# engyasin/EKF-MonoSLAM_for_3D-reconstruction

Hardware: AMD Instinct MI355X
Metric: EKF updates/sec at N features (state dim 14+6N) (higher is better)
Workload: dtype f32 (state, covariance, every accumulation and every other contraction in fp32; the products of the covariance downdate as 3 x bf16 splits of the fp32 operands, six bf16 products per fp32 product: the dropped terms are <= 2^-24 |a||b| in the worst case (2^-28 on average) -- the size of the fp32 prod; 1 GPU; N=1000 inverse-depth features, n=6014, M=N measured per frame, fp32, 1xMI355X (BASELINE configs[2]); features=1000, state_dim=6014, measured_per_frame=1000, camera=conf_kinect.cfg/scale2, frames_per_map=3000, maps=1

## Files before the change

### ekf-monoslam_for_3d-reconstruction_amd/csrc/ekf_capi.hip

```cpp
#include <hip/hip_runtime.h>

#include <algorithm>
#include <array>
#include <climits>
#include <cmath>
#include <cstdint>
#include <cstdio>
#include <cstdlib>
#include <cstring>
#include <map>
#include <mutex>
#include <string>
#include <type_traits>
#include <vector>

#include "../../include/ekf_monoslam.h"
#include "ekf_buffers.hpp"
#include "ekf_feature_table.hpp"
#include "ekf_dense.hpp"
#include "ekf_image.hpp"
#include "ekf_features.hpp"
#include "ekf_syrk6.hpp"
#include "ekf_chain.hpp"
#include "ekf_small.hpp"
// ... 38 lines not shown
  KID_SEED_MASK,
  KID_SEED_RESPONSE,
  KID_SEED_CANDIDATES,
  KID_SEED_SELECT,
  KID_FRAME_UPLOAD,
  KID_FRAME_INGEST,
  KID_FRAME_RECTIFY,
  KID_COUNT
};

static const char* kKernelNames[KID_COUNT] = {
    "predict_camera",  "propagate_strips", "propagate_streaming", "measure",
    "innovation",      "sigma_ht",         "innovation_cov",      "chol_diag",
    "chol_panel",      "chol_trailing",    "state_update",        "downdate_syrk",
    "solve_trmm",      "normalize_quat",  "add_feature",      "compact_transform",   "misc",
    "w_update", "allgather_h", "allgather_s", "allgather_v", "allgather_sigma",
    "seed_mask", "seed_response", "seed_candidates", "seed_select", "frame_upload", "frame_ingest", "frame_rectify"};

static const char* kLaunchNames[EKF_LAUNCH_KINDS] = {
    "downdate_bf16x6", "downdate_f32", "downdate_f32_fused_wu", "downdate_f32_half_tail", "downdate_f32_t64",
    "row_rider", "row_gemv", "row_tile_gemm", "w_update_gemm", "w_recompute",
    "chain_step_launches", "chain_persistent", "solve", "solve_two_groups", "update_oneblock", "update_allinone",
    "chain_trail_diag", "split_image", "state_update_tail", "update_onelaunch", "chain_dist_gather", "chain_step_fused",
    "downdate_mirror_bounds"};

static inline int round_up(int v, int a) { return (v + a - 1) / a * a; }

struct MaskedStreamPool {
  struct Entry { int device, num_cus, reserved; hipStream_t st; };
  std::mutex mu;
  std::vector<Entry> idle;
  bool hooked = false;
  static void at_exit();
  hipStream_t take(int device, int num_cus, int reserved) {
    std::lock_guard<std::mutex> lk(mu);
    for (size_t i = 0; i < idle.size(); ++i)
      if (idle[i].device == device && idle[i].num_cus == num_cus && idle[i].reserved == reserved) {
        hipStream_t st = idle[i].st;
        idle.erase(idle.begin() + i);
        return st;
      }
    return nullptr;
  }
  void give(int device, int num_cus, int reserved, hipStream_t st) {
    std::lock_guard<std::mutex> lk(mu);
    idle.push_back({device, num_cus, reserved, st});
    if (!hooked) { hooked = true; atexit(&MaskedStreamPool::at_exit); }
// ... 169 lines not shown
  bool have_frame = false, have_blur = false;
  DevBuf<unsigned char> d_raw;
  int raw_w = 0, raw_h = 0, raw_c = 0;
  bool have_raw = false;
  RectScratch rect;
  DevBuf<int4> d_ingest_tab;
  int ingest_tab_w = 0, ingest_tab_h = 0;
  DevBuf<unsigned char> d_patch[2], d_mpatch[2];
  int cur_patch = 0;
  DevBuf<T> d_hb, d_zm;
  DevBuf<unsigned char> d_found;
  DevBuf<float> d_score;
  DevBuf<int> d_keep;
  int opt_panel_direct = 1;
  int opt_chain_fused_diag = 1;
  int opt_small_onelaunch = 1;
  int opt_step_fused = 1;
  struct StepPlan { std::vector<int> off, cnt; } sfp;
  WorkList sf_lists{{0}, {}};
  DevBuf<unsigned long long> d_small_stamps;
  unsigned small_gate_total = 0;
  int opt_su_tail = 1;
  int opt_syrk_mirror_skip = 1;
  int opt_fuse_split = 1;
  int opt_chain_defer = 1;
  int td_min_blocks = 24;
  int td_max_blocks = 1 << 30;
  WorkList td_blocks;
  std::vector<int> td_off, td_cnt;
  int opt_syrk_stag_half = 0, opt_syrk_stag_mod4 = 2;
  int opt_solve_s2 = 1;
  bool want_solve_s2(int width, int npad_live) const {
    return kIsF32 && opt_mfma && opt_solve_s2 && (opt_solve_s2 > 1 || (width / 128) * (npad_live / 64) <= 2 * num_cus);
  }
  int opt_fused = 1;
  int opt_solve_one_per_cu = 1;
  int opt_wrecompute = 1;
  int opt_row_gemv = 1;
  int opt_fuse_wu = 1;
  int env_chunks[8] = {}, env_nchunks = 0;
  int opt_pipeline = -1;
  WorkList tilemap{{0, 0}, {}};
  int tri_count = 0, solve_off = 0;
  int w_zeroed_n = -1;
  DevBuf<int> d_counters;
  int num_cus = 256, reserved_cus = 32;
// ... 83 lines not shown
    HIPCHK(d_Hc.reserve(cn * 14));
    HIPCHK(d_Hf.reserve(cn * 12));
    HIPCHK(d_Sd.reserve(cn * 4));
    HIPCHK(d_flags.reserve(cn));
    HIPCHK(d_cflag.reserve(cn));
    HIPCHK(d_trk.reserve(cn));
    HIPCHK(hipMemsetAsync(d_trk, 0, cn, stream));
    HIPCHK(d_Jy.reserve(cn * 18));
    HIPCHK(d_Yxyz.reserve(cn * 3));
    HIPCHK(d_map_src.reserve((size_t)n_pad));
    HIPCHK(d_map_conv.reserve((size_t)n_pad));
    HIPCHK(d_Y.reserve((size_t)2 * ldy * ldy));
    HIPCHK(hipMemsetAsync(d_Y, 0, (size_t)2 * ldy * ldy * sizeof(T), stream));
    HIPCHK(d_W.reserve((size_t)w_rows * ldy));
    HIPCHK(hipMemsetAsync(d_W, 0, (size_t)w_rows * ldy * sizeof(T), stream));
    HIPCHK(d_V.reserve((size_t)w_rows * ldy));
    HIPCHK(hipMemsetAsync(d_V, 0, (size_t)w_rows * ldy * sizeof(T), stream));
    HIPCHK(d_Dinv.reserve((size_t)(ldy / 64) * 128 * 128));
    HIPCHK(d_z.reserve((size_t)ldy));
    HIPCHK(d_midx.reserve(cn));
    HIPCHK(d_status.reserve(16));
    HIPCHK(hipMemsetAsync(d_status, 0, 16 * sizeof(int), stream));
    HIPCHK(d_tmp.reserve(64));
    HIPCHK(d_counters.reserve(kQueueCounters + kMirrorRowsInts));
    HIPCHK(hipMemset(d_counters, 0, (kQueueCounters + kMirrorRowsInts) * sizeof(int)));
    {
      hipDeviceProp_t prop;
      HIPCHK(hipGetDeviceProperties(&prop, device));
      num_cus = prop.multiProcessorCount > 0 ? prop.multiProcessorCount : 256;
    }
    {
      reserved_cus = std::min(32, num_cus / 4);
      if (const char* e = getenv("EKF_RESERVED_CUS")) reserved_cus = std::max(1, std::min(num_cus / 2, atoi(e)));
      std::vector<uint32_t> mask((num_cus + 31) / 32, 0xffffffffu);
      for (int i = 0; i < reserved_cus; ++i) mask[i / 32] &= ~(1u << (i % 32));
      stream_b = g_masked_streams.take(device, num_cus, reserved_cus);
      stream_b_masked = stream_b != nullptr;
      if (!stream_b) {
        if (hipExtStreamCreateWithCUMask(&stream_b, (uint32_t)mask.size(), mask.data()) == hipSuccess) {
          stream_b_masked = true;
        } else {
          (void)hipGetLastError();
          stream_b = nullptr;
          reserved_cus = 0;
          HIPCHK(hipStreamCreateWithFlags(&stream_b, hipStreamNonBlocking));
        }
      }
      stream_b_reserved = reserved_cus;

      if (const char* e = getenv("EKF_FUSE_WU")) opt_fuse_wu = atoi(e);
      if (const char* e = getenv("EKF_ROW_GEMV")) opt_row_gemv = atoi(e) ? 1 : 0;
      if (const char* e = getenv("EKF_SOLVE_ONE_PER_CU")) opt_solve_one_per_cu = atoi(e) ? 1 : 0;
      if (const char* e = getenv("EKF_W_RECOMPUTE")) opt_wrecompute = atoi(e) ? 1 : 0;
      if (const char* e = getenv("EKF_SOLVE_S2")) opt_solve_s2 = atoi(e);
      if (const char* e = getenv("EKF_FUSED_LAUNCHES")) opt_fused = atoi(e) ? 1 : 0;
      if (const char* e = getenv("EKF_PANEL_DIRECT")) opt_panel_direct = atoi(e);
      if (const char* e = getenv("EKF_SYRK_STAGGER")) {
        opt_syrk_stag_half = atoi(e);
        if (const char* c = strchr(e, ',')) opt_syrk_stag_mod4 = atoi(c + 1);
      }
      if (const char* e = getenv("EKF_CHAIN_FUSED_DIAG")) opt_chain_fused_diag = atoi(e) ? 1 : 0;
      if (const char* e = getenv("EKF_FUSE_SPLIT")) opt_fuse_split = atoi(e) ? 1 : 0;
      if (const char* e = getenv("EKF_SU_TAIL")) opt_su_tail = atoi(e) ? 1 : 0;
      if (const char* e = getenv("EKF_SYRK_MIRROR_SKIP")) opt_syrk_mirror_skip = atoi(e) ? 1 : 0;
      if (const char* e = getenv("EKF_SMALL_ONELAUNCH")) opt_small_onelaunch = atoi(e) ? 1 : 0;
      if (const char* e = getenv("EKF_STEP_FUSED")) opt_step_fused = atoi(e) ? 1 : 0;
      if (const char* e = getenv("EKF_SHARD_DIST_CHAIN")) opt_shard_dist_chain = atoi(e) ? 1 : 0;
      if (const char* e = getenv("EKF_SHARD_DIST_MIN_BLOCKS")) shard_dist_min_blocks = std::max(2, atoi(e));
      if (const char* e = getenv("EKF_SMALL_STAMPS")) {
        if (atoi(e)) { HIPCHK(d_small_stamps.reserve(16)); HIPCHK(hipMemset(d_small_stamps, 0, 16 * sizeof(unsigned long long))); }
      }
      if (const char* e = getenv("EKF_CHAIN_DEFER")) opt_chain_defer = atoi(e) ? 1 : 0;
      if (const char* e = getenv("EKF_TD_MIN_BLOCKS")) td_min_blocks = std::max(1, atoi(e));
      if (const char* e = getenv("EKF_TD_MAX_BLOCKS")) td_max_blocks = std::max(1, atoi(e));
      if (const char* e = getenv("EKF_SPLIT_TAIL")) opt_split_tail = atoi(e);
      if (const char* e = getenv("EKF_SPLIT_BF16")) opt_split_bf16 = atoi(e) ? 1 : 0;
      if (const char* e = getenv("EKF_CHUNKS")) {
        for (const char* q = e; *q && env_nchunks < 8;) {
          env_chunks[env_nchunks++] = atoi(q);
          while (*q && *q != ',') ++q;
          if (*q == ',') ++q;
        }
      }
    }
    std::vector<T> mu0(camera_dim, T(0));
    mu0[3] = T(0.0); mu0[4] = T(0.0); mu0[5] = T(-0.707106781); mu0[6] = T(0.707106781);
    if (camera_dim == 14) mu0[13] = T(1);
// ... 788 lines not shown
    if (s2) {
      T* o = static_cast<T*>(s2);
      const T* sd = psd;
      for (int i = 0; i < N; ++i) { o[4 * i] = sd[4 * i]; o[4 * i + 1] = sd[4 * i + 2]; o[4 * i + 2] = sd[4 * i + 1]; o[4 * i + 3] = sd[4 * i + 3]; }
    }
    if (hc) { T* o = static_cast<T*>(hc); for (int i = 0; i < N; ++i) for (int a = 0; a < 2; ++a) for (int c = 0; c < 7; ++c) o[14 * i + c * 2 + a] = vhc[14 * i + a * 7 + c]; }
    if (hf) { T* o = static_cast<T*>(hf); for (int i = 0; i < N; ++i) for (int a = 0; a < 2; ++a) for (int c = 0; c < 6; ++c) o[12 * i + c * 2 + a] = vhf[12 * i + a * 6 + c]; }
    return EKF_OK;
  }

  struct GemmCall {
    const T* A = nullptr; int lda = 0;
    const T* B = nullptr; int ldb = 0;
    T* C = nullptr; int ldc = 0;
    int rows = 0, cols = 0, K = 0;
    T alpha = T(1), beta = T(0);
    int tri = TRI_ALL, row_off = 0, col_off = 0, ktri = KTRI_FULL, ktile_off = 0;
    int zrow = 0, zcol_end = 0;
    const int* tile_list = nullptr; int ntiles = 0;
    int* counter = nullptr;
    void* img = nullptr; int img_nkc = 0, img_c0 = 0;
    bool two_groups = false;
    bool one_per_cu = false;
    hipStream_t st = nullptr;
  };
  struct Rows { int r0, count; };
  struct UpdatePlan {
    int M = 0, plane = 0;
    int nb = 0, tile = 0, m = 0, m_pad = 0, npad_live = 0, nsteps = 0;
    int nchunks = 1, cend[8] = {};
    ChunkTab tab{};
    int strip_rows = 0;
    int ntr = 0, ntc = 0;
    bool oneblock = false, allinone = false, onelaunch = false;
    int small_rc = 0, small_nchunk = 0, small_nt64 = 0;
    bool recompute = false;
    int r0 = 0, r1 = 0, p0 = 0, prows = 0;
    Rows ranges[3] = {};
    bool sym_panel = false, shard_split = false;
    int c0(int g) const { return (g ? cend[g - 1] : 0) * nb; }
    int c1(int g) const { return cend[g] * nb; }
  };
  struct UpdateCtx {
    const T* z;
    const int* midx;
    int* counters;
    int counter_next = 0;
    bool step_fused = false;
    int diag_ahead = -1;
    struct { int step = -1, c0 = 0, c1 = 0; } pending;
    bool row_pending = false;
    bool queue_room(int ints = 8) const { return counter_next + ints <= kQueueCounters; }
    int* take_queue() {
      if (!queue_room()) return nullptr;
      counter_next += 8;
      return counters + counter_next - 8;
    }
  };

  template <int ROLE, bool BT, int TM = 128, int TN = 128>
  void gemm(const GemmCall& c) {
    GemmArgs g{};
    g.A = c.A; g.lda = c.lda; g.B = c.B; g.ldb = c.ldb; g.C = c.C; g.ldc = c.ldc;
    g.K = c.K; g.alpha = double(c.alpha); g.beta = double(c.beta);
    g.tri = c.tri; g.row_off = c.row_off; g.col_off = c.col_off; g.ktri = c.ktri; g.ktile_off = c.ktile_off;
    g.zrow = c.zrow; g.zcol_end = c.zcol_end;
    g.stagger = (ROLE == ROLE_DOWNDATE) ? 1 : 0;
    g.img = c.img; g.img_nkc = c.img_nkc; g.img_c0 = c.img_c0;
    hipStream_t st = c.st ? c.st : stream;
    const bool mf = kIsF32 && opt_mfma;
    dim3 grid(c.cols / (mf ? TN : 64), c.rows / (mf ? TM : 64));
    if (c.tile_list && c.counter) {
      g.tile_map = c.tile_list;
      g.ntiles = c.ntiles;
      g.counter = c.counter;
      const bool side = (st == stream_b);
      int wgs = 2 * (side ? (num_cus - reserved_cus) : num_cus);
      if (ROLE == ROLE_SOLVE && c.one_per_cu) wgs = num_cus;
      grid = dim3(std::min(c.ntiles, wgs), 1);
    }
    if constexpr (kIsF32) {
      if (opt_mfma) {
        if constexpr (ROLE == ROLE_SOLVE) {
          ++launch_cnt[c.two_groups ? EKF_LAUNCH_SOLVE_TWO_GROUPS : EKF_LAUNCH_SOLVE];
          if (c.two_groups) {
            k_gemm_mfma<ROLE, BT, TM, TN, true><<<grid, 512, 0, st>>>(g);
            return;
          }
        }
        k_gemm_mfma<ROLE, BT, TM, TN><<<grid, 256, 0, st>>>(g);
        return;
// ... 133 lines not shown
      *strip_rows = std::max(*strip_rows, (cend[g] - (g ? cend[g - 1] : 0)) * nb);
    }
    return tab;
  }

  int build_innovation(const T* zp, const int* ip, int M, int plane, bool with_nu, int* m_out, int* m_pad_out,
                       const ChunkTab* tab = nullptr, int strip_rows = 0, bool w_only = false) {
    const int nb = NB();
    const int m = 2 * M + (plane ? 3 : 0);
    const int m_pad = round_up(m, nb);
    const int npad_live = round_up(n, nb);
    T* nu_row = d_W + (size_t)ldy * npad_live;
    if (w_zeroed_n != n) {
      HIPCHK(hipMemsetAsync(d_W + (size_t)n * ldy, 0, (size_t)(npad_live - n + nb) * ldy * sizeof(T), stream));
      w_zeroed_n = n;
    }
    const bool small = (size_t)n * m_pad < ((size_t)1 << 22);
    {
      Scope sc(this, KID_SIGMA_HT);
      const int extra = with_nu ? 1 : 0;
      const T* zq = with_nu ? zp : nullptr;
      T* nuq = with_nu ? nu_row : nullptr;
      const ChunkTab st = tab ? *tab : ChunkTab{0, {}};
      int* mrows = (with_nu && tab) ? d_counters + kQueueCounters : nullptr;
      if (small) {
        constexpr int RB = 4;
        dim3 grid((m_pad / 2 + 255) / 256, (n + RB - 1) / RB + extra);
        k_sigma_ht<T, RB><<<grid, 256, 0, stream>>>(S(), ld, n, d_Hc, d_Hf, d_pos, d_coding, ip, M, plane, d_W, ldy,
                                                  m_pad, 0, n, N, zq, d_h, mu(), nuq, d_counters, d_status, d_scr + SCR_QOLD, 0, 0, st, mrows);
      } else if constexpr (kIsF32) {
        constexpr int RB = 8;
        dim3 grid((m_pad / 2 + 127) / 128, (n + RB - 1) / RB + extra);
        k_sigma_ht_fast<RB><<<grid, 256, 0, stream>>>(S(), ld, n, d_Hc, d_Hf, d_pos, d_coding, ip, M, plane, d_W, ldy, m_pad, N,
                                                      0, 0, zq, d_h, mu(), nuq, d_counters, d_status, d_scr + SCR_QOLD, 0, st, mrows);
      } else {
        constexpr int RB = 32;
        dim3 grid((m_pad / 2 + 255) / 256, (n + RB - 1) / RB + extra);
        k_sigma_ht<T, RB><<<grid, 256, 0, stream>>>(S(), ld, n, d_Hc, d_Hf, d_pos, d_coding, ip, M, plane, d_W, ldy,
                                                  m_pad, 0, n, N, zq, d_h, mu(), nuq, d_counters, d_status, d_scr + SCR_QOLD, 0, 0, st, mrows);
      }
    }
    if (!w_only) {
      Scope sc(this, KID_INNOVATION_COV);
      T* zid = tab ? d_Y + (size_t)m_pad * ldy : nullptr;
      const ChunkTab ct = tab ? *tab : ChunkTab{0, {}};
      if (small) {
        constexpr int KB = 1;
// ... 321 lines not shown
        int rc = ensure_step_fused_lists(p.nsteps);
        if (rc) return rc;
        ux.step_fused = true;
      }
    }
    return EKF_OK;
  }

  bool chunk_overlaps(const UpdatePlan& p, int g) const { return stream_b != nullptr && g + 1 < p.nchunks; }
  int chunk_slots(const UpdatePlan& p, int g) const { return 2 * (chunk_overlaps(p, g) ? num_cus - reserved_cus : num_cus); }
  bool chunk_splits(const UpdatePlan& p, const UpdateCtx& ux) const {
    return kIsF32 && opt_split_bf16 && opt_mfma && p.tile == 128 && tri_count >= num_cus && ux.queue_room();
  }
  bool chunk_fuses(const UpdatePlan& p, int g, const UpdateCtx& ux) const {
    return kIsF32 && opt_fuse_wu && (opt_fuse_wu > 1 || p.recompute || g + 2 < p.nchunks) && opt_mfma && chunk_overlaps(p, g) &&
           p.c1(g) < p.m_pad && !opt_split_bf16 && p.tile == 128 && tri_count >= num_cus && ux.queue_room();
  }
  bool chunk_row_rider(const UpdatePlan& p, int g, const UpdateCtx& ux) const {
    return chunk_splits(p, ux) && p.recompute && opt_row_gemv && p.c1(g) < p.m_pad && !chunk_fuses(p, g, ux);
  }
  bool chunk_su_tail(const UpdatePlan& p, int g, const UpdateCtx& ux) const {
    return kIsF32 && opt_su_tail && !chunk_overlaps(p, g) && p.nchunks > 1 && chunk_splits(p, ux);
  }
  enum SolveShape { SOLVE_64X64, SOLVE_128_ONE_PER_CU, SOLVE_64X128, SOLVE_128 };
  SolveShape solve_shape(const UpdatePlan& p, int g) const {
    const bool mf = kIsF32 && opt_mfma;
    const int tiles = (p.c1(g) - p.c0(g)) / p.tile * p.ntr, slots = chunk_slots(p, g);
    if (mf && 4 * tiles < slots) return SOLVE_64X64;
    if (mf && !chunk_overlaps(p, g) && opt_solve_one_per_cu && tiles < slots && tiles > num_cus) return SOLVE_128_ONE_PER_CU;
    if (mf && tiles < slots) return SOLVE_64X128;
    return SOLVE_128;
  }

  int launch_update_small(const UpdatePlan& p, const UpdateCtx& ux) {
    if constexpr (kIsF32) {
      if (w_zeroed_n != n) {
        HIPCHK(hipMemsetAsync(d_W + (size_t)n * ldy, 0, (size_t)(p.npad_live - n + p.nb) * ldy * sizeof(T), stream));
        w_zeroed_n = n;
      }
      SmallUpdateArgs a{};
      a.S = S(); a.ld = ld; a.n = n; a.npad = p.npad_live;
      a.Hc = d_Hc; a.Hf = d_Hf; a.pos = d_pos; a.coding = d_coding; a.midx = ux.midx;
      a.M = p.M; a.plane = p.plane; a.nfeat = N;
      a.z = ux.z; a.h = d_h; a.mu = mu();
      a.r_pix = T(sigma_pixel_2); a.r_plane = T(0.00001);
      a.W = d_W; a.ldw = ldy; a.Y = d_Y; a.ldy = ldy; a.Dinv = d_Dinv; a.V = d_V; a.ldv = ldy;
// ... 11 lines not shown

  int solve_chunk(const UpdatePlan& p, int gi, UpdateCtx& ux, hipStream_t ss, bool* vimg_done) {
    const int c0 = p.c0(gi), width = p.c1(gi) - c0, ntr = p.ntr, ntc = p.ntc;
    T* Zs = d_Y + (size_t)p.m_pad * ldy;
    if (p.oneblock) {
      if constexpr (kIsF32) {
        ++launch_cnt[p.allinone ? EKF_LAUNCH_UPDATE_ALLINONE : EKF_LAUNCH_UPDATE_ONEBLOCK];
        if (p.allinone)
          k_update_oneblock_small<<<p.small_nt64 + 1, 512, 0, ss>>>(d_W, ldy, d_Dinv, d_V, ldy, p.npad_live, mu(), n, d_scr + SCR_QOLD,
                                                                   d_scr + SCR_QN, Zs, ldy, S(), ld, p.small_nt64);
        else
          k_solve_state_oneblock<<<p.npad_live / 64 + 1, 256, 0, ss>>>(d_W, ldy, d_Dinv, d_V, ldy, p.npad_live, mu(), n,
                                                                      d_scr + SCR_QN, Zs, ldy);
      }
      return EKF_OK;
    }
    Scope sc(this, KID_SOLVE, ss);
    const int wt = width / p.tile;
    GemmCall c;
    c.A = d_W + c0; c.lda = ldy; c.B = Zs + c0; c.ldb = ldy; c.C = d_V + c0; c.ldc = ldy;
    c.rows = p.npad_live + p.nb; c.cols = width; c.K = width; c.ktri = KTRI_UPPER;
    c.two_groups = want_solve_s2(width, p.npad_live);
    c.st = ss;
    switch (solve_shape(p, gi)) {
      case SOLVE_64X64:
        c.tile_list = tilemap.d + solve6464_off + 2 * (2 * ntc - 2 * wt) * 2 * ntr; c.ntiles = 2 * wt * 2 * ntr;
        c.counter = ux.take_queue();
        gemm<ROLE_SOLVE, true, 64, 64>(c);
        break;
      case SOLVE_128_ONE_PER_CU:
        c.tile_list = tilemap.d + solve_off + 2 * (ntc - wt) * ntr; c.ntiles = wt * ntr;
        c.counter = ux.take_queue();
        c.one_per_cu = true;
        gemm<ROLE_SOLVE, true>(c);
        break;
      case SOLVE_64X128:
        if (kIsF32 && opt_fuse_split && opt_split_bf16 && p.tile == 128 && tri_count >= num_cus && ux.queue_room(16)) {
          HIPCHK(ensure_vimg());
          c.img = d_Vimg; c.img_nkc = ldy / 16; c.img_c0 = c0;
          *vimg_done = true;
        }
        c.tile_list = tilemap.d + solve64_off + 2 * (ntc - wt) * 2 * ntr; c.ntiles = wt * 2 * ntr;
        c.counter = ux.take_queue();
        gemm<ROLE_SOLVE, true, 64, 128>(c);
        break;
      case SOLVE_128:
// ... 11 lines not shown
    if (p.recompute) {
      launch_row_update(c0, c1, p.m_pad, ss, kIsF32 && opt_row_gemv);
      return;
    }
    Scope sc(this, KID_WUPDATE, ss);
    ++launch_cnt[EKF_LAUNCH_W_UPDATE_GEMM];
    GemmCall c;
    c.A = d_V + c0; c.lda = ldy; c.B = d_Y + (size_t)c1 * ldy + c0; c.ldb = ldy; c.C = d_W + c1; c.ldc = ldy;
    c.rows = p.npad_live + p.nb; c.cols = p.m_pad - c1; c.K = c1 - c0; c.alpha = T(-1); c.beta = T(1);
    c.st = ss;
    if (kIsF32 && opt_mfma && ((p.m_pad - c1) / 128) * p.ntr < chunk_slots(p, gi))
      gemm<ROLE_WUPDATE, false, 64, 128>(c);
    else
      gemm<ROLE_WUPDATE, false>(c);
  }

  int downdate_chunk(const UpdatePlan& p, int gi, UpdateCtx& ux, hipStream_t ss, bool vimg_done) {
    const int c0 = p.c0(gi), c1 = p.c1(gi), width = c1 - c0, m = p.m, m_pad = p.m_pad, npad_live = p.npad_live;
    if (chunk_splits(p, ux)) {
      const bool row_rider = chunk_row_rider(p, gi, ux), su_tail = chunk_su_tail(p, gi, ux);
      if (!vimg_done) ++launch_cnt[EKF_LAUNCH_SPLIT_IMAGE];
      const int* mirror_rows = nullptr;
      if (opt_syrk_mirror_skip && gi + 1 < p.nchunks)
        mirror_rows = d_counters + kQueueCounters + 2 * (p.recompute ? gi + 1 : kMirrorEmpty);
      return launch_downdate_bf16x6(ux, c0, c1, m_pad, ss, !vimg_done, tilemap.d + tri6_off, tri_count, 0, 0, INT_MAX,
                                    double(n) * n * (std::min(c1, m) - std::min(c0, m)), row_rider, su_tail, mirror_rows);
    }
    if (chunk_fuses(p, gi, ux)) {
      if constexpr (kIsF32) {
        Scope sc(this, KID_DOWNDATE, ss);
        const int nr2 = p.recompute ? 1 : (npad_live + p.nb) / 128, n2 = nr2 * ((m_pad - c1) / 128);
        if (sc.on) {
          const double w = std::min(c1, m) - std::min(c0, m);
          prof.work[KID_DOWNDATE] += double(n) * n * w + 2.0 * (p.recompute ? 1 : n + 1) * std::max(0, m - c1) * w;
        }
        GemmArgs g{};
        g.A = d_V + c0; g.lda = ldy; g.B = d_V + c0; g.ldb = ldy; g.C = S(); g.ldc = ld;
        g.K = width; g.alpha = -1.0; g.beta = 1.0; g.tri = TRI_LOWER_MIRROR;
        g.tile_map = tilemap.d; g.ntiles = n2 + tri_count; g.counter = ux.take_queue(); g.stagger = 1;
        g.B2 = d_Y + (size_t)c1 * ldy + c0; g.ldb2 = ldy; g.C2 = d_W + c1; g.ldc2 = ldy;
        g.n2 = n2; g.nr2 = nr2; g.row2 = p.recompute ? npad_live / 128 : 0;
        ++launch_cnt[EKF_LAUNCH_DOWNDATE_F32_FUSED_WU];
        const int wgs = 2 * (num_cus - reserved_cus);
        k_gemm_mfma<ROLE_DOWNDATE, false><<<std::min(g.ntiles, wgs), 256, 0, ss>>>(g);
      }
      return EKF_OK;
    }
// ... 60 lines not shown
    rc = ensure_tilemap(p.npad_live / p.tile, p.ntr, p.ntc);
    if (rc) return rc;
    rc = prepare_chain(p, ux, false);
    if (rc) return rc;
    const int nchunks = p.nchunks, m_pad = p.m_pad;
    bool b_inflight = false;
    for (int gi = 0; gi < (p.onelaunch ? 0 : nchunks); ++gi) {
      const int c0 = p.c0(gi), c1 = p.c1(gi);
      chain_steps(ux, gi ? p.cend[gi - 1] : 0, p.cend[gi], c0, c1, p.m, m_pad, stream, p.oneblock,
                  opt_chain_defer && gi + 1 < nchunks);
      const bool overlap = chunk_overlaps(p, gi);
      hipStream_t ss = overlap ? stream_b : stream;
      if (!overlap && b_inflight) {
        if (p.recompute) {
          HIPCHK(hipEventRecord(ev_b, stream_b));
          HIPCHK(hipStreamWaitEvent(stream, ev_b, 0));
          b_inflight = false;
        } else {
          HIPCHK(hipStreamWaitEvent(stream, ev_wu, 0));
        }
      }
      if (overlap) {
        b_inflight = true;
        HIPCHK(hipEventRecord(ev_chain[gi], stream));
        HIPCHK(hipStreamWaitEvent(stream_b, ev_chain[gi], 0));
      }
      bool vimg_done = false;
      rc = solve_chunk(p, gi, ux, ss, &vimg_done);
      if (rc) return rc;
      const bool fuse = chunk_fuses(p, gi, ux);
      wupdate_chunk(p, gi, ux, ss);
      if (overlap && c1 < m_pad && !fuse && !p.recompute) HIPCHK(hipEventRecord(ev_wu, stream_b));
      if (!overlap && b_inflight) {
        HIPCHK(hipEventRecord(ev_b, stream_b));
        HIPCHK(hipStreamWaitEvent(stream, ev_b, 0));
        b_inflight = false;
      }
      if (!overlap && nchunks > 1 && !chunk_su_tail(p, gi, ux)) {
        HIPCHK(hipEventRecord(ev_chain[gi], stream));
        HIPCHK(hipStreamWaitEvent(stream_b, ev_chain[gi], 0));
        launch_state_update(m_pad, stream_b);
        b_inflight = true;
      }
      rc = downdate_chunk(p, gi, ux, ss, vimg_done);
      if (rc) return rc;
      if (fuse && !p.recompute) HIPCHK(hipEventRecord(ev_wu, stream_b));
      if (p.recompute && gi + 1 < nchunks) {
        launch_w_recompute(c1, p.c1(gi + 1), m_pad, ux.midx, M, plane, ss, n);
// ... 3496 lines not shown
```

### ekf-monoslam_for_3d-reconstruction_amd/csrc/ekf_dense.hpp

```cpp
#pragma once
#include <type_traits>
#include "ekf_math.hpp"

namespace ekf {

typedef float f32x4 __attribute__((ext_vector_type(4)));
constexpr int kQueueCounters = 256;

__device__ __forceinline__ int clamp_feature(int fi, int nfeat) { return min(max(fi, 0), nfeat - 1); }
__device__ __forceinline__ void check_measured_entry(const int* __restrict__ midx, int k, int nfeat,
                                                     int* __restrict__ status) {
  const int fi = midx[k];
  if (status && (fi < 0 || fi >= nfeat || (k > 0 && midx[k - 1] >= fi))) status[1] = 1;
}

struct ChunkTab {
  int n;
  int end[8];
};

constexpr int kMirrorEmpty = 8;
constexpr int kMirrorRowsInts = 2 * (kMirrorEmpty + 1);
__device__ __forceinline__ void mirror_rows_slab(const ChunkTab& tab, const int* __restrict__ midx, int M, int nfeat,
                                                 const int* __restrict__ pos, const int* __restrict__ coding,
                                                 int* __restrict__ mrows) {
  __shared__ int s_lo[8], s_hi[8];
  const int tid = threadIdx.x;
  if (tid < 8) { s_lo[tid] = 0x7fffffff; s_hi[tid] = 0; }
  __syncthreads();
  for (int k = tid; k < M; k += blockDim.x) {
    int g = 0;
#pragma unroll
    for (int u = 0; u < 7; ++u)
      if (u + 1 < tab.n && 2 * k >= tab.end[u]) g = u + 1;
    const int fi = clamp_feature(midx[k], nfeat);
    const int p = pos[fi];
    atomicMin(&s_lo[g], p);
    atomicMax(&s_hi[g], p + (coding[fi] ? 3 : 6));
  }
  __syncthreads();
  if (tid <= kMirrorEmpty) {
    const bool some = tid < 8 && s_hi[tid & 7] > s_lo[tid & 7];
    mrows[2 * tid] = some ? s_lo[tid] : 0;
    mrows[2 * tid + 1] = some ? s_hi[tid] : 0;
  }
}

template <typename T>
__global__ void k_innovation(const T* __restrict__ z, const T* __restrict__ h, const int* __restrict__ midx,
                             int M, int plane, const T* __restrict__ mu, T* __restrict__ nu, int m_pad,
                             int* __restrict__ counters, int nfeat, int* __restrict__ status) {
  const int t = blockIdx.x * blockDim.x + threadIdx.x;
  if (counters)
    for (int c = t; c < kQueueCounters; c += gridDim.x * blockDim.x) counters[c] = 0;
  if (t >= m_pad) return;
  T v = T(0);
  if (t < 2 * M) {
    if ((t & 1) == 0) check_measured_entry(midx, t >> 1, nfeat, status);
    v = z[t] - h[2 * clamp_feature(midx[t >> 1], nfeat) + (t & 1)];
  } else if (plane && t < 2 * M + 3) {
    const int e = t - 2 * M;
    v = -mu[e == 0 ? 1 : (e == 1 ? 4 : 6)];
  }
  nu[t] = v;
}

template <typename T, int RB>
__global__ void k_sigma_ht(const T* __restrict__ S, int ld, int n,
                           const T* __restrict__ Hc, const T* __restrict__ Hf,
                           const int* __restrict__ pos, const int* __restrict__ coding,
                           const int* __restrict__ midx, int M, int plane,
                           T* __restrict__ W, int ldy, int m_pad, int row_begin, int row_end,
                           int nfeat,
                           const T* __restrict__ z = nullptr, const T* __restrict__ h = nullptr,
                           const T* __restrict__ mu = nullptr, T* __restrict__ nu = nullptr,
                           int* __restrict__ counters = nullptr, int* __restrict__ status = nullptr,
                           T* __restrict__ q_old = nullptr, int slot0 = 0, int slot_end = 0,
                           ChunkTab tab = ChunkTab{0, {}}, int* __restrict__ mirror_rows = nullptr) {
  const int k = slot0 + blockIdx.x * blockDim.x + threadIdx.x;
  const int nslots = slot_end > 0 ? slot_end : m_pad / 2;
  if (nu != nullptr && blockIdx.y == gridDim.y - 1) {
    if (q_old && k < 4) q_old[k] = mu[3 + k];
    if (counters)
      for (int c = k; c < kQueueCounters; c += gridDim.x * blockDim.x) counters[c] = 0;
    if (mirror_rows && blockIdx.x == 0) mirror_rows_slab(tab, midx, M, nfeat, pos, coding, mirror_rows);
    if (k >= nslots) return;
    if (k < M) check_measured_entry(midx, k, nfeat, status);
#pragma unroll
    for (int t = 2 * k; t < 2 * k + 2; ++t) {
      T v = T(0);
      if (t < 2 * M) {
        v = z[t] - h[2 * clamp_feature(midx[t >> 1], nfeat) + (t & 1)];
      } else if (plane && t < 2 * M + 3) {
        const int e = t - 2 * M;
        v = -mu[e == 0 ? 1 : (e == 1 ? 4 : 6)];
      }
      nu[t] = v;
    }
    return;
  }
  const int row0 = row_begin + blockIdx.y * RB;
  if (k >= nslots) return;
  const int row1 = min(row0 + RB, min(row_end, n));
  if (k < M) {
    const int fi = clamp_feature(midx[k], nfeat);
    const int p = pos[fi];
    const int fs = coding[fi] ? 3 : 6;
// ... 55 lines not shown

template <int RB>
__global__ void __launch_bounds__(256, RB <= 8 ? 6 : 3)
k_sigma_ht_fast(const float* __restrict__ S, int ld, int n,
                const float* __restrict__ Hc, const float* __restrict__ Hf,
                const int* __restrict__ pos, const int* __restrict__ coding,
                const int* __restrict__ midx, int M, int plane,
                float* __restrict__ W, int ldy, int m_pad, int nfeat, int slot0, int slot_end,
                const float* __restrict__ z, const float* __restrict__ h, const float* __restrict__ mu,
                float* __restrict__ nu, int* __restrict__ counters, int* __restrict__ status, float* __restrict__ q_old,
                int row_lo = 0,
                ChunkTab tab = ChunkTab{0, {}}, int* __restrict__ mirror_rows = nullptr) {
  constexpr int SL = 128, SEG = 6 * SL + 4;
  typedef float f4 __attribute__((ext_vector_type(4)));
  typedef float f2 __attribute__((ext_vector_type(2)));
  __shared__ __attribute__((aligned(16))) float seg[RB * SEG];
  __shared__ __attribute__((aligned(16))) float cam[RB * 8];
  const int tid = threadIdx.x;
  if (nu != nullptr && blockIdx.y == gridDim.y - 1) {
    const int k = blockIdx.x * blockDim.x + tid;
    const int nslots = m_pad / 2;
    if (q_old && k < 4) q_old[k] = mu[3 + k];
    if (counters)
      for (int c = k; c < kQueueCounters; c += gridDim.x * blockDim.x) counters[c] = 0;
    if (mirror_rows && blockIdx.x == 0) mirror_rows_slab(tab, midx, M, nfeat, pos, coding, mirror_rows);
    if (k >= nslots) return;
    if (k < M) check_measured_entry(midx, k, nfeat, status);
#pragma unroll
    for (int t = 2 * k; t < 2 * k + 2; ++t) {
      float v = 0.f;
      if (t < 2 * M) {
        v = z[t] - h[2 * clamp_feature(midx[t >> 1], nfeat) + (t & 1)];
      } else if (plane && t < 2 * M + 3) {
        const int e = t - 2 * M;
        v = -mu[e == 0 ? 1 : (e == 1 ? 4 : 6)];
      }
      nu[t] = v;
    }
    return;
  }
  const int s = tid & (SL - 1), half = tid >> 7;
  const int kbase = slot0 + blockIdx.x * SL;
  const int k = kbase + s;
  const int nslots = slot_end > 0 ? slot_end : m_pad / 2;
  const int row0 = row_lo + blockIdx.y * RB, row1 = min(row0 + RB, n);
  int fi = -1, p = 0, fs = 6;
  if (k < M && k < nslots) {
// ... 173 lines not shown
    }
  }
}

enum : int { ROLE_PANEL = 0, ROLE_TRAILING = 1, ROLE_DOWNDATE = 2, ROLE_SOLVE = 3, ROLE_GAIN = 4, ROLE_WUPDATE = 5 };
enum : int { TRI_ALL = 0, TRI_LOWER = 1, TRI_LOWER_MIRROR = 2, TRI_LISTED = 3 };
enum : int { KTRI_FULL = 0, KTRI_UPPER = 1 };

struct GemmArgs {
  const void* A; int lda;
  const void* B; int ldb;
  void* C; int ldc;
  int K;
  double alpha, beta;
  int tri, row_off, col_off, ktri, ktile_off;
  const int* tile_map; int ntiles; int* counter;
  int zrow, zcol_end;
  int stagger;
  const void* B2; int ldb2;
  void* C2; int ldc2;
  int n2, nr2;
  int row2;
  void* img = nullptr; int img_nkc = 0, img_c0 = 0;
};
constexpr int kSecondProduct = 0x10000;
constexpr int kHalfTile = 0x20000;
constexpr int kMirrorTile = 0x40000;

__device__ __forceinline__ bool gemm_next_tile(const GemmArgs& g, int* s_tile, int& iter, int& bi, int& bj) {
  if (!g.tile_map) {
    if (iter++) return false;
    bi = blockIdx.y;
    bj = blockIdx.x;
    return true;
  }
  __syncthreads();
  if (threadIdx.x == 0) {
    *s_tile = atomicAdd(g.counter, 1);
  }
  __syncthreads();
  const int t = __builtin_amdgcn_readfirstlane(*s_tile);
  if (t >= g.ntiles) return false;
  if (t < g.n2) {
    bi = g.row2 + t % g.nr2;
    bj = (t / g.nr2) | kSecondProduct;
  } else {
    bi = g.tile_map[2 * (t - g.n2)];
// ... 78 lines not shown

template <int ROLE, bool BT, int TM = 128, int TN = 128, bool S2 = false>
__global__ void __launch_bounds__(S2 ? 512 : 256, S2 ? 1 : ((ROLE == ROLE_TRAILING && TM == 64 && TN == 64) ? 6 : 2)) k_gemm_mfma(GemmArgs g) {
  constexpr int NT = 256, WC = 2, BK = 32, NQ = BK / 4, NJ = TN / (32 * WC), PB = TN * 8 / NT;
  constexpr bool SPLIT = (ROLE == ROLE_DOWNDATE) && !BT && TM == 128 && TN == 128;
  static_assert((TM == 64 || TM == 128) && (TN == 64 || TN == 128), "tile shape");
  const float* A = static_cast<const float*>(g.A);
  const float* B0 = static_cast<const float*>(g.B);
  float* C0 = static_cast<float*>(g.C);
  const int lda = g.lda;
  constexpr bool DUAL = (ROLE == ROLE_DOWNDATE) && !BT && TM == 128 && TN == 128;
  const float alpha = float(g.alpha), beta = float(g.beta);
  __shared__ f32x4 lds[(S2 ? 2 : 1) * 2 * NQ * (TM + TN)];
  int* const s_tile_p = reinterpret_cast<int*>(lds);
  constexpr int STAGE = NQ * (TM + TN);
  const int tid = S2 ? (threadIdx.x & 255) : threadIdx.x;
  const int grp = S2 ? __builtin_amdgcn_readfirstlane(threadIdx.x >> 8) : 0;
  const int lbase = S2 ? grp * 2 * STAGE : 0;
  const int lane = tid & 63, wave = tid >> 6;
  const int wr = wave / WC, wc = wave % WC;
  if (ROLE == ROLE_PANEL || ROLE == ROLE_TRAILING) __builtin_amdgcn_s_setprio(2);
  if (g.stagger && g.tile_map && blockIdx.x >= gridDim.x / 2)
    for (int i = 0; i < g.stagger; ++i) __builtin_amdgcn_s_sleep(127);
  int bi, bj, iter = 0;
  while (gemm_next_tile(g, s_tile_p, iter, bi, bj)) {
  bool listed_mirror = false;
  auto tile_body = [&](auto tm_tag) {
  constexpr int TMb = decltype(tm_tag)::value, MI = TMb / 64, PA = TMb * 8 / NT;
  const bool second = DUAL && (bj & kSecondProduct);
  if (DUAL) bj &= kSecondProduct - 1;
  const float* B = second ? static_cast<const float*>(g.B2) : B0;
  float* C = second ? static_cast<float*>(g.C2) : C0;
  const int ldb = second ? g.ldb2 : g.ldb, ldc = second ? g.ldc2 : g.ldc;
  const int tri = second ? 0 : g.tri;
  const int grow0 = g.row_off + bi * TMb, gcol0 = g.col_off + bj * TN;
  if (tri && tri != 3 && grow0 + TMb <= gcol0) return;
  if (g.zrow && grow0 >= g.zrow && gcol0 >= g.zcol_end) return;
  const int Kall = g.ktri ? min(g.K, (bj + g.ktile_off + 1) * TN) : g.K;
  const int K = S2 ? Kall / 2 : Kall;
  const int koff = S2 ? grp * BK : 0;
  const float* Ag[PA];
  const float* Bg[4];
  int aslot[PA], bslot[4];
#pragma unroll
  for (int p = 0; p < PA; ++p) {
    const int idx = tid + NT * p;
// ... 1461 lines not shown
```

### include/ekf_monoslam.h

```cpp
#ifndef EKF_MONOSLAM_H_
#define EKF_MONOSLAM_H_

#include <stddef.h>

#ifdef __cplusplus
extern "C" {
#endif

#define EKF_ABI_VERSION 6

typedef struct ekf_filter ekf_filter;

enum ekf_dtype { EKF_F32 = 0, EKF_F64 = 1 };

enum ekf_status {
  EKF_OK = 0,
  EKF_ERR_ARG = 1,
  EKF_ERR_CAPACITY = 2,
  EKF_ERR_DEVICE = 3,
  EKF_ERR_STATE = 4,
  EKF_ERR_NUMERIC = 5,
  EKF_ERR_UNSUPPORTED = 6
};

// ... 117 lines not shown
  EKF_LAUNCH_DOWNDATE_BF16X6 = 0,
  EKF_LAUNCH_DOWNDATE_F32,
  EKF_LAUNCH_DOWNDATE_F32_FUSED_WU,
  EKF_LAUNCH_DOWNDATE_F32_HALF_TAIL,
  EKF_LAUNCH_DOWNDATE_F32_T64,
  EKF_LAUNCH_ROW_RIDER,
  EKF_LAUNCH_ROW_GEMV,
  EKF_LAUNCH_ROW_TILE_GEMM,
  EKF_LAUNCH_W_UPDATE_GEMM,
  EKF_LAUNCH_W_RECOMPUTE,
  EKF_LAUNCH_CHAIN_STEP,
  EKF_LAUNCH_CHAIN_PERSISTENT,
  EKF_LAUNCH_SOLVE,
  EKF_LAUNCH_SOLVE_TWO_GROUPS,
  EKF_LAUNCH_UPDATE_ONEBLOCK,
  EKF_LAUNCH_UPDATE_ALLINONE,
  EKF_LAUNCH_CHAIN_TRAIL_DIAG,
  EKF_LAUNCH_SPLIT_IMAGE,
  EKF_LAUNCH_STATE_UPDATE_TAIL,
  EKF_LAUNCH_UPDATE_ONELAUNCH,
  EKF_LAUNCH_CHAIN_DIST_GATHER,
  EKF_LAUNCH_CHAIN_STEP_FUSED,
  EKF_LAUNCH_DOWNDATE_MIRROR_BOUNDS,
  EKF_LAUNCH_KINDS
};
int ekf_launch_kinds(void);
const char* ekf_launch_kind_name(int kind);
int ekf_launch_count(ekf_filter* f, int kind, long long* launches);

typedef int (*ekf_allgather_fn)(void* ctx, const void* d_send, void* d_recv, size_t bytes_per_rank, void* hip_stream);

typedef struct ekf_shard_info {
  int rank, world, N, state_dim;
  int f_begin, f_end;
  int row_begin, row_end;
  int max_rows_any_rank;
  int rebalances;
} ekf_shard_info;

int ekf_shard_configure(ekf_filter* f, int rank, int world, ekf_allgather_fn allgather, void* ctx);
int ekf_shard_get_info(ekf_filter* f, ekf_shard_info* out);
int ekf_shard_update(ekf_filter* f, const void* d_z, const int* indices, int M, int plane_constraint);
int ekf_shard_rebalance(ekf_filter* f);

void* ekf_device_mu(ekf_filter* f);
void* ekf_device_sigma(ekf_filter* f, int* ld);
// ... 144 lines not shown
```

Measured before the change: 1145 updates/s.

## Replace cross-stream event wait with device-side epoch polling in chunked solve

For overlapped chunks on the CU-masked second stream, the solve kernel no longer waits on a hipEvent recorded on the main stream. Instead, a tiny kernel on the main stream atomically publishes an epoch word, and the solve kernel's first thread spin-polls that word with an acquire fence before starting tiles. The aim is to remove the host/driver latency of the event-based cross-stream dependency so the solve can launch early. In exchange, solve blocks occupy CUs while spinning, and a timeout path flags an error status. The counter reset range is widened to cover the epoch word.

```diff
diff --git a/ekf-monoslam_for_3d-reconstruction_amd/csrc/ekf_capi.hip b/ekf-monoslam_for_3d-reconstruction_amd/csrc/ekf_capi.hip
--- a/ekf-monoslam_for_3d-reconstruction_amd/csrc/ekf_capi.hip
+++ b/ekf-monoslam_for_3d-reconstruction_amd/csrc/ekf_capi.hip
@@ -84,7 +84,7 @@
     "row_rider", "row_gemv", "row_tile_gemm", "w_update_gemm", "w_recompute",
     "chain_step_launches", "chain_persistent", "solve", "solve_two_groups", "update_oneblock", "update_allinone",
     "chain_trail_diag", "split_image", "state_update_tail", "update_onelaunch", "chain_dist_gather", "chain_step_fused",
-    "downdate_mirror_bounds"};
+    "downdate_mirror_bounds", "solve_poll_chain"};
 
 static inline int round_up(int v, int a) { return (v + a - 1) / a * a; }
 
@@ -300,6 +300,7 @@
   unsigned small_gate_total = 0;
   int opt_su_tail = 1;
   int opt_syrk_mirror_skip = 1;
+  int opt_solve_poll_chain = 1;
   int opt_fuse_split = 1;
   int opt_chain_defer = 1;
   int td_min_blocks = 24;
@@ -429,8 +430,8 @@
     HIPCHK(d_status.reserve(16));
     HIPCHK(hipMemsetAsync(d_status, 0, 16 * sizeof(int), stream));
     HIPCHK(d_tmp.reserve(64));
-    HIPCHK(d_counters.reserve(kQueueCounters + kMirrorRowsInts));
-    HIPCHK(hipMemset(d_counters, 0, (kQueueCounters + kMirrorRowsInts) * sizeof(int)));
+    HIPCHK(d_counters.reserve(kResetInts + kMirrorRowsInts));
+    HIPCHK(hipMemset(d_counters, 0, (kResetInts + kMirrorRowsInts) * sizeof(int)));
     {
       hipDeviceProp_t prop;
       HIPCHK(hipGetDeviceProperties(&prop, device));
@@ -470,6 +471,7 @@
       if (const char* e = getenv("EKF_FUSE_SPLIT")) opt_fuse_split = atoi(e) ? 1 : 0;
       if (const char* e = getenv("EKF_SU_TAIL")) opt_su_tail = atoi(e) ? 1 : 0;
       if (const char* e = getenv("EKF_SYRK_MIRROR_SKIP")) opt_syrk_mirror_skip = atoi(e) ? 1 : 0;
+      if (const char* e = getenv("EKF_SOLVE_POLL_CHAIN")) opt_solve_poll_chain = std::max(0, std::min(2, atoi(e)));
       if (const char* e = getenv("EKF_SMALL_ONELAUNCH")) opt_small_onelaunch = atoi(e) ? 1 : 0;
       if (const char* e = getenv("EKF_STEP_FUSED")) opt_step_fused = atoi(e) ? 1 : 0;
       if (const char* e = getenv("EKF_SHARD_DIST_CHAIN")) opt_shard_dist_chain = atoi(e) ? 1 : 0;
@@ -1304,6 +1306,7 @@
     void* img = nullptr; int img_nkc = 0, img_c0 = 0;
     bool two_groups = false;
     bool one_per_cu = false;
+    const unsigned* chain_word = nullptr; unsigned chain_epoch = 0;
     hipStream_t st = nullptr;
   };
   struct Rows { int r0, count; };
@@ -1349,6 +1352,7 @@
     g.zrow = c.zrow; g.zcol_end = c.zcol_end;
     g.stagger = (ROLE == ROLE_DOWNDATE) ? 1 : 0;
     g.img = c.img; g.img_nkc = c.img_nkc; g.img_c0 = c.img_c0;
+    g.chain_word = c.chain_word; g.chain_epoch = c.chain_epoch; g.status = d_status;
     hipStream_t st = c.st ? c.st : stream;
     const bool mf = kIsF32 && opt_mfma;
     dim3 grid(c.cols / (mf ? TN : 64), c.rows / (mf ? TM : 64));
@@ -1528,7 +1532,7 @@
       const T* zq = with_nu ? zp : nullptr;
       T* nuq = with_nu ? nu_row : nullptr;
       const ChunkTab st = tab ? *tab : ChunkTab{0, {}};
-      int* mrows = (with_nu && tab) ? d_counters + kQueueCounters : nullptr;
+      int* mrows = (with_nu && tab) ? d_counters + kResetInts : nullptr;
       if (small) {
         constexpr int RB = 4;
         dim3 grid((m_pad / 2 + 255) / 256, (n + RB - 1) / RB + extra);
@@ -1896,6 +1900,10 @@
   bool chunk_su_tail(const UpdatePlan& p, int g, const UpdateCtx& ux) const {
     return kIsF32 && opt_su_tail && !chunk_overlaps(p, g) && p.nchunks > 1 && chunk_splits(p, ux);
   }
+  bool solve_polls_chain(const UpdatePlan& p, int g) const {
+    return kIsF32 && opt_mfma && opt_solve_poll_chain && (p.nsteps <= 16 || opt_solve_poll_chain > 1) && g > 0 &&
+           chunk_overlaps(p, g) && stream_b_masked && reserved_cus > 0 && !p.oneblock;
+  }
   enum SolveShape { SOLVE_64X64, SOLVE_128_ONE_PER_CU, SOLVE_64X128, SOLVE_128 };
   SolveShape solve_shape(const UpdatePlan& p, int g) const {
     const bool mf = kIsF32 && opt_mfma;
@@ -1953,6 +1961,10 @@
     c.rows = p.npad_live + p.nb; c.cols = width; c.K = width; c.ktri = KTRI_UPPER;
     c.two_groups = want_solve_s2(width, p.npad_live);
     c.st = ss;
+    if (ss == stream_b && solve_polls_chain(p, gi)) {
+      c.chain_word = reinterpret_cast<const unsigned*>(d_counters + kChainEpochWord); c.chain_epoch = (unsigned)gi + 1;
+      ++launch_cnt[EKF_LAUNCH_SOLVE_POLL_CHAIN];
+    }
     switch (solve_shape(p, gi)) {
       case SOLVE_64X64:
         c.tile_list = tilemap.d + solve6464_off + 2 * (2 * ntc - 2 * wt) * 2 * ntr; c.ntiles = 2 * wt * 2 * ntr;
@@ -2010,7 +2022,7 @@
       if (!vimg_done) ++launch_cnt[EKF_LAUNCH_SPLIT_IMAGE];
       const int* mirror_rows = nullptr;
       if (opt_syrk_mirror_skip && gi + 1 < p.nchunks)
-        mirror_rows = d_counters + kQueueCounters + 2 * (p.recompute ? gi + 1 : kMirrorEmpty);
+        mirror_rows = d_counters + kResetInts + 2 * (p.recompute ? gi + 1 : kMirrorEmpty);
       return launch_downdate_bf16x6(ux, c0, c1, m_pad, ss, !vimg_done, tilemap.d + tri6_off, tri_count, 0, 0, INT_MAX,
                                     double(n) * n * (std::min(c1, m) - std::min(c0, m)), row_rider, su_tail, mirror_rows);
     }
@@ -2117,8 +2129,13 @@
       }
       if (overlap) {
         b_inflight = true;
-        HIPCHK(hipEventRecord(ev_chain[gi], stream));
-        HIPCHK(hipStreamWaitEvent(stream_b, ev_chain[gi], 0));
+        if (solve_polls_chain(p, gi)) {
+          if constexpr (kIsF32)
+            k_publish_epoch<<<1, 64, 0, stream>>>(reinterpret_cast<unsigned*>(d_counters + kChainEpochWord), (unsigned)gi + 1);
+        } else {
+          HIPCHK(hipEventRecord(ev_chain[gi], stream));
+          HIPCHK(hipStreamWaitEvent(stream_b, ev_chain[gi], 0));
+        }
       }
       bool vimg_done = false;
       rc = solve_chunk(p, gi, ux, ss, &vimg_done);
diff --git a/ekf-monoslam_for_3d-reconstruction_amd/csrc/ekf_dense.hpp b/ekf-monoslam_for_3d-reconstruction_amd/csrc/ekf_dense.hpp
--- a/ekf-monoslam_for_3d-reconstruction_amd/csrc/ekf_dense.hpp
+++ b/ekf-monoslam_for_3d-reconstruction_amd/csrc/ekf_dense.hpp
@@ -6,6 +6,8 @@
 
 typedef float f32x4 __attribute__((ext_vector_type(4)));
 constexpr int kQueueCounters = 256;
+constexpr int kChainEpochWord = kQueueCounters;
+constexpr int kResetInts = kQueueCounters + 32;
 
 __device__ __forceinline__ int clamp_feature(int fi, int nfeat) { return min(max(fi, 0), nfeat - 1); }
 __device__ __forceinline__ void check_measured_entry(const int* __restrict__ midx, int k, int nfeat,
@@ -52,7 +54,7 @@
                              int* __restrict__ counters, int nfeat, int* __restrict__ status) {
   const int t = blockIdx.x * blockDim.x + threadIdx.x;
   if (counters)
-    for (int c = t; c < kQueueCounters; c += gridDim.x * blockDim.x) counters[c] = 0;
+    for (int c = t; c < kResetInts; c += gridDim.x * blockDim.x) counters[c] = 0;
   if (t >= m_pad) return;
   T v = T(0);
   if (t < 2 * M) {
@@ -82,7 +84,7 @@
   if (nu != nullptr && blockIdx.y == gridDim.y - 1) {
     if (q_old && k < 4) q_old[k] = mu[3 + k];
     if (counters)
-      for (int c = k; c < kQueueCounters; c += gridDim.x * blockDim.x) counters[c] = 0;
+      for (int c = k; c < kResetInts; c += gridDim.x * blockDim.x) counters[c] = 0;
     if (mirror_rows && blockIdx.x == 0) mirror_rows_slab(tab, midx, M, nfeat, pos, coding, mirror_rows);
     if (k >= nslots) return;
     if (k < M) check_measured_entry(midx, k, nfeat, status);
@@ -184,7 +186,7 @@
     const int nslots = m_pad / 2;
     if (q_old && k < 4) q_old[k] = mu[3 + k];
     if (counters)
-      for (int c = k; c < kQueueCounters; c += gridDim.x * blockDim.x) counters[c] = 0;
+      for (int c = k; c < kResetInts; c += gridDim.x * blockDim.x) counters[c] = 0;
     if (mirror_rows && blockIdx.x == 0) mirror_rows_slab(tab, midx, M, nfeat, pos, coding, mirror_rows);
     if (k >= nslots) return;
     if (k < M) check_measured_entry(midx, k, nfeat, status);
@@ -404,7 +406,12 @@
   int n2, nr2;
   int row2;
   void* img = nullptr; int img_nkc = 0, img_c0 = 0;
+  const unsigned* chain_word = nullptr; unsigned chain_epoch = 0; int* status = nullptr;
 };
+
+__global__ void k_publish_epoch(unsigned* word, unsigned epoch) {
+  if (threadIdx.x == 0) __hip_atomic_store(word, epoch, __ATOMIC_RELAXED, __HIP_MEMORY_SCOPE_AGENT);
+}
 constexpr int kSecondProduct = 0x10000;
 constexpr int kHalfTile = 0x20000;
 constexpr int kMirrorTile = 0x40000;
@@ -529,6 +536,21 @@
   if (ROLE == ROLE_PANEL || ROLE == ROLE_TRAILING) __builtin_amdgcn_s_setprio(2);
   if (g.stagger && g.tile_map && blockIdx.x >= gridDim.x / 2)
     for (int i = 0; i < g.stagger; ++i) __builtin_amdgcn_s_sleep(127);
+  if constexpr (ROLE == ROLE_SOLVE) {
+    if (g.chain_word != nullptr) {
+      if (threadIdx.x == 0) {
+        bool ok = false;
+        for (int spin = 0; spin < (1 << 20) && !ok; ++spin) {
+          ok = (int)(__hip_atomic_load(g.chain_word, __ATOMIC_RELAXED, __HIP_MEMORY_SCOPE_AGENT) - g.chain_epoch) >= 0;
+          if (!ok) __builtin_amdgcn_s_sleep(8);
+        }
+        if (!ok) g.status[3] = 1;
+        __builtin_amdgcn_fence(__ATOMIC_ACQUIRE, "agent");
+        asm volatile("s_waitcnt vmcnt(0)" ::: "memory");
+      }
+      __syncthreads();
+    }
+  }
   int bi, bj, iter = 0;
   while (gemm_next_tile(g, s_tile_p, iter, bi, bj)) {
   bool listed_mirror = false;
diff --git a/include/ekf_monoslam.h b/include/ekf_monoslam.h
--- a/include/ekf_monoslam.h
+++ b/include/ekf_monoslam.h
@@ -163,6 +163,7 @@
   EKF_LAUNCH_CHAIN_DIST_GATHER,
   EKF_LAUNCH_CHAIN_STEP_FUSED,
   EKF_LAUNCH_DOWNDATE_MIRROR_BOUNDS,
+  EKF_LAUNCH_SOLVE_POLL_CHAIN,
   EKF_LAUNCH_KINDS
 };
 int ekf_launch_kinds(void);
```

Result: faster. 1160 updates/s, median of 6 (+1.3%).
